# deflect-ca/banjax

Hardware: AMD Instinct MI355X
Metric: log lines/sec matched+rate-limited (node) at 1k rules; HBM GB/s vs peak (higher is better)
Workload: dtype u8

## Files before the change

banjax_amd/csrc/engine.hip:

```cpp
#include <hip/hip_runtime.h>
#include <hipcub/hipcub.hpp>

#include <algorithm>
#include <array>
#include <atomic>
#include <cstdio>
#include <cstdlib>
#include <cstring>
#include <map>
#include <tuple>
#include <memory>
#include <mutex>
#include <stdexcept>
#include <string>
#include <unordered_map>
#include <thread>
#include <vector>

#include "../../include/banjax_gpu.h"
#include "bjx_common.h"
#include "engine_types.h"
#include "regex_compiler.h"
#include "bans.h"

using namespace bjx;

namespace {

struct BjxError : std::runtime_error {
  int code;
  BjxError(int c, const std::string &m) : std::runtime_error(m), code(c) {}
};

#define HIP_OK(expr)                                                                                   \
  do {                                                                                                 \
    hipError_t e_ = (expr);                                                                            \
    if (e_ != hipSuccess)                                                                              \
      throw BjxError(BJX_ERR_DEVICE, std::string(#expr " failed: ") + hipGetErrorString(e_));          \
  } while (0)

constexpr int kBlock = 256;



__device__ __forceinline__ uint32_t nl_mask_word(uint32_t v) {
  uint32_t x = v ^ 0x0A0A0A0Au;
  uint32_t t = ((x & 0x7F7F7F7Fu) + 0x7F7F7F7Fu) | x;
  return ~t & 0x80808080u;
}


__device__ __forceinline__ uint32_t find_space(const uint8_t *p, uint32_t i, uint32_t n) {
  while (i < n && p[i] != ' ') ++i;
  return i;
}

__device__ __forceinline__ bool bytes_eq(const uint8_t *a, const uint8_t *b, uint32_t n) {
  uint32_t k = 0;
  for (; k + 4 <= n; k += 4)
    if (ld4(a + k) != ld4(b + k)) return false;
  for (; k < n; ++k)
    if (a[k] != b[k]) return false;
  return true;
}

__device__ __forceinline__ uint4 ip_key16(const uint8_t *ip, uint32_t len) {
  uint32_t w[4];
#pragma unroll
  for (int k = 0; k < 4; ++k) {
    const uint32_t lo = 4u * k;
    const uint32_t m = len <= lo ? 0u : (len >= lo + 4 ? 0xFFFFFFFFu : (1u << (8 * (len - lo))) - 1u);
    w[k] = m ? ld4(ip + lo) & m : 0u;
  }
  w[3] = (w[3] & 0x00FFFFFFu) | ((len < 255 ? len : 255u) << 24);
  return make_uint4(w[0], w[1], w[2], w[3]);
}
__device__ __forceinline__ uint4 ip_key16_bytes(const uint8_t *ip, uint32_t len) {
  uint32_t w[4] = {0, 0, 0, 0};
  for (uint32_t k = 0; k < len && k < 15; ++k) w[k >> 2] |= (uint32_t)ip[k] << (8 * (k & 3));
  w[3] |= (len < 255 ? len : 255u) << 24;
  return make_uint4(w[0], w[1], w[2], w[3]);
}
constexpr uint32_t kIpWords = 12;

template <uint32_t NW>
__device__ __forceinline__ void ip_words(const uint8_t *p, uint32_t n, uint32_t (&w)[NW]) {
  const uint32_t sh = (uint32_t)(reinterpret_cast<uintptr_t>(p) & 3);
  const uint32_t *a = reinterpret_cast<const uint32_t *>(p - sh);
  const uint32_t nw = n ? (sh + n + 3) >> 2 : 0u;
  uint32_t r[NW + 1];
#pragma unroll
  for (uint32_t k = 0; k <= NW; ++k) r[k] = k < nw ? a[k] : 0u;
#pragma unroll
  for (uint32_t k = 0; k < NW; ++k) {
    const uint32_t lo = 4u * k;
    const uint32_t m = n <= lo ? 0u : (n >= lo + 4 ? 0xFFFFFFFFu : (1u << (8 * (n - lo))) - 1u);
    w[k] = __builtin_amdgcn_alignbyte(r[k + 1], r[k], sh) & m;
  }
}
template <uint32_t NW>
__device__ __forceinline__ uint64_t hash_words(const uint32_t (&w)[NW], uint32_t n) {
// ... 348 lines not shown
    } else if (rule_match(B, r, rest, rest_len)) {
      word |= 1ull << (pos & 63);
      ++nres;
      nev += is_skip(B, r, hid) ? 0u : 1u;
    }
    ++pos;
    if ((pos & 63) == 0) { L.mword(j, wi++) = word; word = 0; }
  }
  if (pos & 63) L.mword(j, wi) = word;
  L.counts[j] = ((uint64_t)nres << 32) | nev;
}

__global__ void k_no_line_pass(unsigned long long *slow_count, unsigned long long n) {
  if (threadIdx.x == 0) *slow_count = n;
}

template <bool SLOW>
__global__ __launch_bounds__(kBlock) void k_parse_match(Bind B, const uint8_t *__restrict__ buf,
                                                        const uint64_t *__restrict__ nl, uint64_t n_lines,
                                                        const uint32_t *__restrict__ list, int64_t now_ns, Lines L,
                                                        uint32_t *slow_list, unsigned long long *slow_count, WideList WL) {
  const uint64_t t = (uint64_t)blockIdx.x * blockDim.x + threadIdx.x;
  if (t >= n_lines) return;
  const uint64_t j = SLOW && list ? list[t] : t;
  const uint64_t s = j ? nl[j - 1] + 1 : 0;
  const uint32_t n = (uint32_t)(nl[j] - s);
  parse_and_match<SLOW>(B, buf + s, s, n, j, now_ns, L, slow_list, slow_count, WL);
}


constexpr uint32_t kWT = 4096;
constexpr uint32_t kHalo = 512;
constexpr uint32_t kLineCap = 128;
constexpr uint32_t kHitSlots = 4;
constexpr int kScanWaves = 16;
constexpr uint32_t kTileLds = kWT + kHalo + 16;
constexpr uint32_t kWaveJobs = 64;
constexpr int kScanGroup = 8;
constexpr uint32_t kCandList = 128;
constexpr uint32_t kBanChunks = 8;
constexpr uint64_t kBanChunkMin = 64ull << 20;
constexpr uint32_t kLongList = 64;
constexpr uint32_t kWaveLds = kTileLds + kLineCap * (2 + 2) + kCandList * 4 + kLineCap * 4 + kLongList * 8 + 16;
constexpr uint32_t kNone = 0xFFFFFFFFu;
constexpr uint32_t kScanLdsMax = 160 * 1024;
constexpr uint32_t kLinesImgMax = 16 * 1024;
constexpr uint32_t kLinesHostLdsMax = 6 * 1024;
constexpr uint32_t kLinesTabLdsMax = 10 * 1024;
constexpr uint32_t kLinesBlocksPerCu = 3;
constexpr uint32_t kSpanBytes = 12 * 1024;

__device__ __forceinline__ uint32_t space_mask16(const uint4 v) {
  const uint32_t wv[4] = {v.x, v.y, v.z, v.w};
  uint32_t m16 = 0;
#pragma unroll
  for (int k = 0; k < 4; ++k) {
    const uint32_t x = wv[k] ^ 0x20202020u;
    const uint32_t hb = ~(((x & 0x7F7F7F7Fu) + 0x7F7F7F7Fu) | x) & 0x80808080u;
    m16 |= (((hb >> 7) & 1u) | ((hb >> 14) & 2u) | ((hb >> 21) & 4u) | ((hb >> 28) & 8u)) << (4 * k);
  }
  return m16;
}

__device__ __forceinline__ bool digits4(uint32_t x) {
  return (x & 0xF0F0F0F0u) == 0x30303030u && (((x & 0x0F0F0F0Fu) + 0x06060606u) & 0xF0F0F0F0u) == 0u;
}
__device__ __forceinline__ uint32_t value4(uint32_t x) {
  x -= 0x30303030u;
  x = x * 10u + (x >> 8);
  return (x & 0xFFu) * 100u + ((x >> 16) & 0xFFu);
}
__device__ __forceinline__ int parse_ts_msec(const uint8_t *p, uint32_t n, double *out) {
  if (n != 14) return 1;
  const uint32_t w0 = ld4(p), w1 = ld4(p + 4), w2 = ld4(p + 8), w3 = ld4(p + 12);
  if (!digits4(w0) || !digits4(w1) || (w2 & 0x00FF0000u) != 0x002E0000u || !digits4((w2 & 0xFF00FFFFu) | 0x00300000u) ||
      !digits4((w3 & 0xFFFFu) | 0x30300000u))
    return 1;
  const uint32_t d8 = w2 & 0xFFu, d9 = (w2 >> 8) & 0xFFu, d11 = w2 >> 24, d12 = w3 & 0xFFu, d13 = (w3 >> 8) & 0xFFu;
  const uint64_t ip = (uint64_t)value4(w0) * 1000000ull + value4(w1) * 100u + (d8 - 48u) * 10u + (d9 - 48u);
  const uint64_t m = ip * 1000ull + (d11 - 48u) * 100u + (d12 - 48u) * 10u + (d13 - 48u);
  *out = (double)m / 1000.0;
  return 0;
}

__device__ __forceinline__ uint32_t find_spaces(const uint8_t *p, uint32_t n, uint32_t &sp0, uint32_t &sp1,
                                                uint32_t &sp2, uint32_t &sp3) {
  const uint32_t skip = (uint32_t)(reinterpret_cast<uintptr_t>(p) & 15);
  const uint4 *base = reinterpret_cast<const uint4 *>(p - skip);
  uint32_t ns = 0, c0 = 0;
  if (n + skip >= 64) {
    const uint4 v0 = base[0], v1 = base[1], v2 = base[2], v3 = base[3];
    uint64_t m = (uint64_t)space_mask16(v0) | ((uint64_t)space_mask16(v1) << 16) | ((uint64_t)space_mask16(v2) << 32) |
                 ((uint64_t)space_mask16(v3) << 48);
    m &= ~((1ull << skip) - 1ull);
#pragma unroll
    for (int k = 0; k < 4; ++k) {
      const uint32_t pos = (uint32_t)__ffsll((unsigned long long)m) - 1 - skip;
      const bool has = m != 0;
      m &= m - 1;
      if (k == 0) sp0 = has ? pos : sp0;
      if (k == 1) sp1 = has ? pos : sp1;
      if (k == 2) sp2 = has ? pos : sp2;
      if (k == 3) sp3 = has ? pos : sp3;
      ns += has ? 1u : 0u;
    }
    c0 = 4;
  }
  for (uint32_t c = c0; c * 16 < n + skip && ns < 4; ++c) {
    const uint4 v = base[c];
    uint32_t m16 = 0;
    const uint32_t wv[4] = {v.x, v.y, v.z, v.w};
#pragma unroll
    for (int k = 0; k < 4; ++k) {
      const uint32_t x = wv[k] ^ 0x20202020u;
      const uint32_t hb = ~(((x & 0x7F7F7F7Fu) + 0x7F7F7F7Fu) | x) & 0x80808080u;
      m16 |= (((hb >> 7) & 1u) | ((hb >> 14) & 2u) | ((hb >> 21) & 4u) | ((hb >> 28) & 8u)) << (4 * k);
    }
    const int32_t lo = (int32_t)skip - (int32_t)(c * 16), hi = lo + (int32_t)n;
    if (lo > 0) m16 &= ~((1u << lo) - 1u);
    if (hi < 16) m16 &= hi > 0 ? (1u << hi) - 1u : 0u;
    while (m16 && ns < 4) {
      const uint32_t pos = c * 16 + (uint32_t)__ffs(m16) - 1 - skip;
      m16 &= m16 - 1;
      sp0 = ns == 0 ? pos : sp0;
      sp1 = ns == 1 ? pos : sp1;
      sp2 = ns == 2 ? pos : sp2;
      sp3 = ns == 3 ? pos : sp3;
      ++ns;
    }
  }
  return ns;
}

struct ScanArgs {
  const uint8_t *buf;
  uint64_t n;
  uint64_t n_tiles;
  uint64_t n_lines;
  const uint64_t *tile_base;
  uint64_t *nl;
  Lines L;
  unsigned long long *stats;
  uint32_t shared_bytes;
  uint32_t debug_skip;
};

__global__ __launch_bounds__(kBlock) void k_nl_count_wt(const uint8_t *__restrict__ buf, uint64_t n, uint64_t n_tiles,
                                                        uint32_t *__restrict__ counts) {
  const uint64_t t = (uint64_t)blockIdx.x * (kBlock / 64) + (threadIdx.x >> 6);
  if (t >= n_tiles) return;
  const uint32_t lane = threadIdx.x & 63;
  const uint64_t base = t * kWT + lane * 64u;
  uint32_t c = 0;
  if (base + 64 <= n) {
    const uint4 *src = reinterpret_cast<const uint4 *>(buf + base);
#pragma unroll
    for (int k = 0; k < 4; ++k) {
      const uint4 v = src[k];
      c += __popc(nl_mask_word(v.x)) + __popc(nl_mask_word(v.y)) + __popc(nl_mask_word(v.z)) + __popc(nl_mask_word(v.w));
    }
  } else {
    for (uint64_t k = base; k < n && k < base + 64; ++k) c += buf[k] == '\n';
  }
  for (int o = 32; o > 0; o >>= 1) c += __shfl_xor(c, o);
  if (lane == 0) counts[t] = c;
}

__device__ __forceinline__ void push_list(uint32_t *list, unsigned long long *count, uint64_t j) {
  const unsigned long long k = atomicAdd(count, 1ull);
  list[k] = (uint32_t)j;
// ... 1561 lines not shown
    const uint32_t aw = acc ? acc[st] : 0u;
    if (aw >> 31) {
      for (;;) {
        uint32_t m = accel_mask(v, aw) & ~((1u << skip) - 1u);
        if (end - a < 16) m &= (1u << (uint32_t)(end - a)) - 1u;
        if (m) { skip = (uint32_t)__ffs(m) - 1; break; }
        a += 16;
        skip = 0;
        if (a >= end) return B.accept_end[R.ae_off + st] != 0;
        v = load16(a);
      }
    }
    const uint4 vn = a + 16 < end ? load16(a + 16) : make_uint4(0, 0, 0, 0);
    const uint32_t wv[4] = {v.x, v.y, v.z, v.w};
    const uint32_t lim = end - a < 16 ? (uint32_t)(end - a) : 16u;
#pragma unroll
    for (uint32_t k = 0; k < 16; ++k) {
      if (k < skip || k >= lim) continue;
      const uint32_t b = (wv[k >> 2] >> (8 * (k & 3))) & 0xFF;
      if (b >= 0x80) {
        const DevRule *Rp = &R;
        uint64_t i = a + k;
        while (i < end) {
          int w;
          const int32_t rune = decode_rune_hd(buf + i, (uint32_t)(end - i), &w);
          uint32_t c;
          if (rune < 0x80) c = ac[rune];
          else {
            const uint32_t *na = B.nonascii + 2 * Rp->na_off;
            uint32_t lo = 0, hi = Rp->n_na;
            while (hi - lo > 1) {
              const uint32_t m = (lo + hi) >> 1;
              if (na[2 * m] <= (uint32_t)rune) lo = m; else hi = m;
            }
            c = na[2 * lo + 1];
          }
          i += (uint32_t)w;
          st = tr[st * ncls + c];
          if (st <= 1) break;
        }
        return B.accept_end[R.ae_off + st] != 0;
      }
      st = tr[st * ncls + ac[b]];
      if (st <= 1) return st == kAccept;
    }
    skip = 0;
    a += 16;
    v = vn;
  }
  return B.accept_end[R.ae_off + st] != 0;
}

__device__ __forceinline__ uint32_t nl_mask16(const uint4 v) {
  const uint32_t wv[4] = {v.x, v.y, v.z, v.w};
  uint32_t m = 0;
#pragma unroll
  for (int q = 0; q < 4; ++q) {
    const uint32_t hb = nl_mask_word(wv[q]);
    m |= (((hb >> 7) & 1u) | ((hb >> 14) & 2u) | ((hb >> 21) & 4u) | ((hb >> 28) & 8u)) << (4 * q);
  }
  return m;
}
template <bool STAGED>
__device__ __forceinline__ bool dfa_line(const Bind &B, const DevRule &R, const uint16_t *tr, const uint8_t *ac,
                                         const uint32_t *acc, const uint8_t *__restrict__ buf, uint64_t n_buf, uint64_t t0,
                                         uint32_t st0) {
  const uint32_t ncls = R.ncls;
  uint32_t st = st0;
  uint64_t a = t0 & ~15ull;
  uint32_t skip = (uint32_t)(t0 - a);
  auto load16 = [&](uint64_t p) -> uint4 {
    if (p + 16 <= n_buf) return *reinterpret_cast<const uint4 *>(buf + p);
    uint32_t w[4];
    for (int k = 0; k < 4; ++k) {
      uint32_t x = 0;
      for (int b = 0; b < 4; ++b) x |= (p + 4 * k + b < n_buf ? (uint32_t)buf[p + 4 * k + b] : 0x0Au) << (8 * b);
      w[k] = x;
    }
    return make_uint4(w[0], w[1], w[2], w[3]);
  };
  uint4 v = load16(a);
  for (;;) {
    uint32_t nlm = nl_mask16(v) & ~((1u << skip) - 1u);
    const uint32_t aw = acc ? acc[st] : 0u;
    if ((aw >> 31) && !nlm) {
      for (;;) {
        const uint32_t m = accel_mask(v, aw) & ~((1u << skip) - 1u);
        if (m || nlm) {
          const uint32_t f = (uint32_t)__ffs(m | nlm) - 1;
          skip = f;
          break;
        }
        a += 16;
        skip = 0;
        v = load16(a);
        nlm = nl_mask16(v);
      }
    } else if (aw >> 31) {
      const uint32_t m = (accel_mask(v, aw) | nlm) & ~((1u << skip) - 1u);
      skip = (uint32_t)__ffs(m) - 1;
    }
    const uint32_t lim = nlm ? (uint32_t)__ffs(nlm) - 1 : 16u;
    const uint4 vn = lim == 16u ? load16(a + 16) : make_uint4(0, 0, 0, 0);
    const uint32_t wv[4] = {v.x, v.y, v.z, v.w};
#pragma unroll
    for (uint32_t k = 0; k < 16; ++k) {
      if (k < skip || k >= lim) continue;
      const uint32_t b = (wv[k >> 2] >> (8 * (k & 3))) & 0xFF;
      if (b >= 0x80) {
        uint64_t i = a + k, end = i;
        while (end < n_buf && buf[end] != '\n') ++end;
        while (i < end) {
          int w;
          const int32_t rune = decode_rune_hd(buf + i, (uint32_t)(end - i), &w);
// ... 4396 lines not shown
                          reinterpret_cast<const void *>(&k_lines<false, false, true>)})
      HIP_OK(hipFuncSetAttribute(f, hipFuncAttributeMaxDynamicSharedMemorySize, (int)kScanLdsMax));
    e->lines_attr = true;
  }
  auto resident_grid = [&](const void *fn, uint32_t lds, uint64_t work) {
    int per_cu = 0;
    HIP_OK(hipOccupancyMaxActiveBlocksPerMultiprocessor(&per_cu, fn, kBlock, lds));
    const uint64_t resident = (uint64_t)std::max(1, per_cu) * (uint64_t)std::max(1, n_cu);
    return (unsigned)std::max<uint64_t>(1, std::min<uint64_t>((work + kBlock - 1) / kBlock, resident));
  };
  for (int attempt = 0;; ++attempt) {
    LinesArgs A;
    A.buf = buf; A.n = n; A.nl = e->nl.p; A.n_lines = n_lines; A.L = L; A.now_ns = now_ns;
    A.dbg = getenv("BJX_DEBUG_LINES") ? (uint32_t)atoi(getenv("BJX_DEBUG_LINES")) : 0u;
    A.dbg2 = getenv("BJX_DEBUG_L2") ? (uint32_t)atoi(getenv("BJX_DEBUG_L2")) : 0u;
    A.slow_list = e->slow_list.p; A.slow_count = e->scalars.p;
    A.jline = e->jline.p; A.jkey = e->jkey.p; A.jidx = e->jidx.p; A.jrec = e->jrec.p; A.job_count = e->scalars.p + 11;
    A.job_cap = std::min(std::min(e->jline.n, e->jkey.n), std::min(e->jidx.n, e->jrec.n));
    A.job_real = e->scalars.p + 14;
    A.null_key = 2 * B.n_rules;
    A.span_bytes = getenv("BJX_SPAN_BYTES") ? (uint32_t)atoi(getenv("BJX_SPAN_BYTES")) & ~15u : kSpanBytes;
    A.list = nullptr; A.n_list = 0; A.prof = nullptr;
    HIP_OK(hipEventRecord(e->evk[0], st));
    static const int lines_env = getenv("BJX_LINES") ? atoi(getenv("BJX_LINES")) : 2;
    const bool use_l2 = B.l2_bytes && lines_env != 1 && !getenv("BJX_PROF_LINES") && !A.dbg;
    e->last_line_kernel = all_wide ? 3u : use_l2 ? 2u : 1u;
    if (all_wide) {
      hipLaunchKernelGGL(k_no_line_pass, dim3(1), dim3(64), 0, st, e->scalars.p, (unsigned long long)n_lines);
      HIP_OK(hipGetLastError());
    } else if (use_l2) {
      const uint32_t lds = B.l2_bytes + (kL2Block / 64) * kL2WaveLds;
      const void *fn = B.l2_w == 2 ? reinterpret_cast<const void *>(&k_lines2<2>) : reinterpret_cast<const void *>(&k_lines2<1>);
      if (lds != e->lines2_lds || B.l2_w != e->lines2_w) {
        HIP_OK(hipFuncSetAttribute(fn, hipFuncAttributeMaxDynamicSharedMemorySize, (int)lds));
        e->lines2_lds = lds;
        e->lines2_w = B.l2_w;
      }
      int per_cu = 0;
      HIP_OK(hipOccupancyMaxActiveBlocksPerMultiprocessor(&per_cu, fn, kL2Block, lds));
      const uint64_t resident = (uint64_t)std::max(1, per_cu) * (uint64_t)std::max(1, n_cu);
      const unsigned grid = (unsigned)std::max<uint64_t>(1, std::min<uint64_t>((n_lines + kL2Block - 1) / kL2Block, resident));
      static const bool dbg_img = getenv("BJX_DEBUG_IMG") != nullptr;
      if (dbg_img) fprintf(stderr, "[bjx] k_lines2: %u B LDS per block (tables %u), %d blocks per CU, grid %u\n", lds, B.l2_bytes, per_cu, grid);
#ifdef BJX_PROF_L2
      e->chk.ensure(16);
      HIP_OK(hipMemsetAsync(e->chk.p, 0, 128, st));
      A.prof = e->chk.p;
#endif
      if (B.l2_w == 2) hipLaunchKernelGGL(k_lines2<2>, dim3(grid), dim3(kL2Block), lds, st, B, A);
      else hipLaunchKernelGGL(k_lines2<1>, dim3(grid), dim3(kL2Block), lds, st, B, A);
      HIP_OK(hipGetLastError());
#ifdef BJX_PROF_L2
      {
        unsigned long long c[8];
        pin_get(e, c, e->chk.p, 64);
        pin_sync(e);
        double tot = 0;
        for (int k = 0; k < 8; ++k) tot += (double)c[k];
        fprintf(stderr, "[bjx] k_lines2 segments (%% of wave clocks): loads %.1f header %.1f host+allow %.1f hits %.1f "
                "anchored %.1f jobs %.1f stores %.1f flush %.1f\n", 100 * c[0] / tot, 100 * c[1] / tot, 100 * c[2] / tot,
                100 * c[3] / tot, 100 * c[4] / tot, 100 * c[5] / tot, 100 * c[6] / tot, 100 * c[7] / tot);
      }
#endif
    } else {
      const bool img_lds = B.img_bytes <= kLinesImgMax;
      const bool host_lds = B.hl_bytes != 0;
      const uint32_t fixed = ((img_lds ? B.img_bytes : 0) + 15u & ~15u) + (host_lds ? B.hl_bytes + 15u & ~15u : 0u) +
                             (kBlock / 64) * kWaveJobBytes;
      if (A.span_bytes && !getenv("BJX_SPAN_BYTES")) {
        const uint32_t share = (kScanLdsMax / kLinesBlocksPerCu) & ~2047u;
        const uint32_t room = share > fixed ? share - fixed : 0u;
        A.span_bytes = std::min<uint32_t>(kSpanBytes, (room / (kBlock / 64) - 32) & ~15u);
      }
      const uint32_t lds = fixed + (kBlock / 64) * (A.span_bytes ? A.span_bytes + 32 : 0);
      const void *fn = img_lds ? (host_lds ? reinterpret_cast<const void *>(&k_lines<true, false, true>)
                                           : reinterpret_cast<const void *>(&k_lines<true>))
                               : (host_lds ? reinterpret_cast<const void *>(&k_lines<false, false, true>)
                                           : reinterpret_cast<const void *>(&k_lines<false>));
      const unsigned grid = resident_grid(fn, lds, A.list ? A.n_list : n_lines);
      const bool prof = getenv("BJX_PROF_LINES") != nullptr;
      A.prof = nullptr;
      if (prof) {
#ifndef BJX_PROF
        throw BjxError(BJX_ERR_ARG, "BJX_PROF_LINES needs a library built with BJX_PROF=1");
#else
        e->chk.ensure(16);
        HIP_OK(hipMemsetAsync(e->chk.p, 0, 128, st));
        A.prof = e->chk.p;
        if (img_lds && host_lds) hipLaunchKernelGGL((k_lines<true, true, true>), dim3(grid), dim3(kBlock), lds, st, B, A);
        else if (img_lds) hipLaunchKernelGGL((k_lines<true, true>), dim3(grid), dim3(kBlock), lds, st, B, A);
        else if (host_lds) hipLaunchKernelGGL((k_lines<false, true, true>), dim3(grid), dim3(kBlock), lds, st, B, A);
        else hipLaunchKernelGGL((k_lines<false, true>), dim3(grid), dim3(kBlock), lds, st, B, A);
        unsigned long long c[10];
        pin_get(e, c, e->chk.p, 80);
        pin_sync(e);
        double tot = 0;
        for (int k = 0; k < 10; ++k) tot += (double)c[k];
        fprintf(stderr, "[bjx] k_lines segments (%% of wave clocks): loads+staging %.1f header %.1f host %.1f host-rules %.1f "
                "hit-decode %.1f site-walk %.1f global-walk %.1f mask-stores %.1f stores %.1f jobs %.1f\n", 100 * c[0] / tot,
                100 * c[1] / tot, 100 * c[2] / tot, 100 * c[3] / tot, 100 * c[7] / tot, 100 * c[8] / tot, 100 * c[9] / tot,
                100 * c[4] / tot, 100 * c[5] / tot, 100 * c[6] / tot);
#endif
      } else if (img_lds && host_lds) hipLaunchKernelGGL((k_lines<true, false, true>), dim3(grid), dim3(kBlock), lds, st, B, A);
      else if (img_lds) hipLaunchKernelGGL(k_lines<true>, dim3(grid), dim3(kBlock), lds, st, B, A);
      else if (host_lds) hipLaunchKernelGGL((k_lines<false, false, true>), dim3(grid), dim3(kBlock), lds, st, B, A);
      else hipLaunchKernelGGL(k_lines<false>, dim3(grid), dim3(kBlock), lds, st, B, A);
      HIP_OK(hipGetLastError());
    }
    HIP_OK(hipEventRecord(e->evk[1], st));
    pin_get(e, &last_nl, e->nl.p + (n_lines - 1), 8);
    pin_get(e, sc4, e->scalars.p + 8, 32);
    pin_get(e, sc4 + 4, e->scalars.p, 8);
    pin_get(e, &n_jobs, e->scalars.p + 14, 8);
    pin_sync(e);
// ... 1219 lines not shown
```

banjax_amd/csrc/lines2.h:

```cpp

#ifdef BJX_PROF_L2
#define L2P(k)                       \
  do {                               \
    __builtin_amdgcn_s_waitcnt(0);   \
    P.mark(k);                       \
  } while (0)
#else
#define L2P(k) \
  do {         \
  } while (0)
#endif

constexpr uint32_t kL2Win = 112;
constexpr int kL2Block = 512;
constexpr uint32_t kL2WaveLds = 64 * kL2Win + kWaveJobBytes;
constexpr uint32_t kL2TabMax = 20 * 1024;
constexpr uint32_t kL2ChkTmpl = 1, kL2ChkFull = 2;
constexpr uint32_t kL2AncWords = 12;
constexpr uint32_t kL2InlineSteps = 64;
constexpr uint32_t kL2NoStart = 0xFFFFFFFFu;
__host__ __device__ constexpr uint32_t l2_dcls_words(uint32_t w) { return (10 * w + 5 + 3) & ~3u; }
__host__ __device__ constexpr uint32_t l2_row_words(uint32_t w) { return (6 * w + 2 + 3) & ~3u; }

template <int W>
struct L2Mask {
  uint64_t w[W];
};
template <int W>
__device__ __forceinline__ L2Mask<W> l2_ld_mask(const uint32_t *hl, uint32_t at) {
  L2Mask<W> m;
#pragma unroll
  for (int k = 0; k < W; ++k) {
    const uint2 v = *reinterpret_cast<const uint2 *>(hl + at + 2 * k);
    m.w[k] = ((uint64_t)v.y << 32) | v.x;
  }
  return m;
}
template <int W>
__device__ __forceinline__ void l2_or(L2Mask<W> &a, const L2Mask<W> &b) {
#pragma unroll
  for (int k = 0; k < W; ++k) a.w[k] |= b.w[k];
}
template <int W>
__device__ __forceinline__ void l2_set(L2Mask<W> &a, uint32_t p) {
#pragma unroll
  for (int k = 0; k < W; ++k)
    if ((p >> 6) == (uint32_t)k) a.w[k] |= 1ull << (p & 63);
}
template <int W>
__device__ __forceinline__ bool l2_has(const L2Mask<W> &a, uint32_t p) {
  bool r = false;
#pragma unroll
  for (int k = 0; k < W; ++k)
    if ((p >> 6) == (uint32_t)k) r = (a.w[k] >> (p & 63)) & 1;
  return r;
}

__device__ __forceinline__ void l2_take_spaces(uint64_t m, int32_t base, uint32_t &ns, uint32_t &sp0, uint32_t &sp1,
                                               uint32_t &sp2, uint32_t &sp3) {
#pragma unroll
  for (int k = 0; k < 4; ++k) {
    const bool has = m != 0 && ns < 4;
    const uint32_t pos = (uint32_t)((int32_t)__ffsll((unsigned long long)m) - 1 + base);
    m &= m - 1;
    sp0 = has && ns == 0 ? pos : sp0;
    sp1 = has && ns == 1 ? pos : sp1;
    sp2 = has && ns == 2 ? pos : sp2;
    sp3 = has && ns == 3 ? pos : sp3;
    ns += has ? 1u : 0u;
  }
}

__device__ __forceinline__ uint32_t l2_spaces(const uint8_t *win, uint32_t sk, const uint8_t *gp, uint32_t n, uint32_t &sp0,
                                              uint32_t &sp1, uint32_t &sp2, uint32_t &sp3) {
  const uint4 *w = reinterpret_cast<const uint4 *>(win);
  uint32_t ns = 0;
  {
    const uint4 v0 = w[0], v1 = w[1], v2 = w[2], v3 = w[3];
    uint64_t m = (uint64_t)space_mask16(v0) | ((uint64_t)space_mask16(v1) << 16) | ((uint64_t)space_mask16(v2) << 32) |
                 ((uint64_t)space_mask16(v3) << 48);
    m &= ~((1ull << sk) - 1ull);
    if (sk + n < 64) m &= (1ull << (sk + n)) - 1ull;
    l2_take_spaces(m, -(int32_t)sk, ns, sp0, sp1, sp2, sp3);
  }
  if (ns < 4 && sk + n > 64) {
    const uint4 v4 = w[4], v5 = w[5], v6 = w[6];
    uint64_t m = (uint64_t)space_mask16(v4) | ((uint64_t)space_mask16(v5) << 16) | ((uint64_t)space_mask16(v6) << 32);
    if (sk + n < kL2Win) m &= (1ull << (sk + n - 64)) - 1ull;
    l2_take_spaces(m, 64 - (int32_t)sk, ns, sp0, sp1, sp2, sp3);
  }
  const uint32_t lim = kL2Win - sk;
  if (ns < 4 && n > lim) {
    uint32_t q0 = 0, q1 = 0, q2 = 0, q3 = 0;
    const uint32_t nq = find_spaces(gp + lim, n - lim, q0, q1, q2, q3);
    const uint32_t q[4] = {q0, q1, q2, q3};
#pragma unroll
    for (uint32_t k = 0; k < 4; ++k) {
      const bool has = k < nq && ns < 4;
      const uint32_t pos = q[k] + lim;
      sp0 = has && ns == 0 ? pos : sp0;
      sp1 = has && ns == 1 ? pos : sp1;
      sp2 = has && ns == 2 ? pos : sp2;
      sp3 = has && ns == 3 ? pos : sp3;
      ns += has ? 1u : 0u;
    }
  }
  return ns;
}

struct L2Line {
  const uint8_t *wp;
  const uint8_t *gp;
  uint32_t lim;
  uint32_t n;
};
__device__ __forceinline__ bool l2_in(const L2Line &X, uint32_t o, uint32_t len) { return o + len + 8 <= X.lim; }

template <bool LDS_TEXT>
__device__ __forceinline__ uint32_t l2_anchored(const Bind &B, const Tabs &T, const LdsTabs &LT, const uint4 a, const uint4 b,
                                                uint32_t r, const uint8_t *rest, uint32_t rest_len, uint32_t host_rel,
                                                uint32_t host_len) {
  const uint32_t kind = (a.x >> 27) & 7u;
  const bool eq = ((a.x >> 30) & 1u) != 0;
  if (kind == kPlanScan) return 2;
  if (kind == kPlanAnchorT) {
    if (!tmpl_at(LT, a.w, rest, rest_len, host_rel, host_len, 0)) return 0;
    return eq ? 1u : 2u;
  }
  const uint4 qa = make_uint4(a.y, a.z, b.x, b.y), qb = make_uint4(b.z, b.w, 0, 0);
  const uint32_t qk = anchor_quick(qa, qb, rest, rest_len);
  if (qk == 0) return 0;
  if (qk == 1 && ((qa.y >> 9) & 1)) return 1;
  if (a.w) {
    if (!((a.w >> 16) <= rest_len && literal_at(T, (a.w & 0xFFFFu) - 1, rest))) return 0;
    return eq ? 1u : 2u;
  }
  const DevRule &R = B.rules[r];
  if (R.anc_len) {
    bool any = false;
    for (uint32_t i = 0; i < R.anc_len && !any; ++i) {
      const uint32_t lit = B.rule_lits[R.anc_off + i];
      any = lit_len_of(T, lit) <= rest_len && literal_at(T, lit, rest);
    }
    if (!any) return 0;
    if (R.anc_equiv) return 1;
  }
  return 2;
}

template <bool LDS_TEXT>
__device__ __forceinline__ uint32_t l2_check(const Tabs &T, const LdsTabs &LT, const uint4 ck, const uint8_t *rest,
                                             uint32_t rest_len, uint32_t host_rel, uint32_t host_len, uint32_t hp) {
  const uint32_t kind = (ck.x >> 8) & 3u;
  const bool eq = ((ck.x >> 10) & 1u) != 0;
  if (kind == kL2ChkTmpl) {
    const uint4 rec = LT.trec[ck.y];
    const uint32_t la = rec.x & 0xFF;
    const bool side_c = ((rec.x >> 16) & 1u) != 0;
// ... 104 lines not shown
    uint4 v = make_uint4(0, 0, 0, 0);
    if (16 - al <= X.n + 1 - o) v = *reinterpret_cast<const uint4 *>(X.gp + o - al);
    else {
      uint32_t t[4] = {0, 0, 0, 0};
      for (uint32_t k = al; k < 16 && o + (k - al) <= X.n; ++k) t[k >> 2] |= (uint32_t)X.gp[o + (k - al)] << (8 * (k & 3));
      v = make_uint4(t[0], t[1], t[2], t[3]);
    }
    const uint32_t w[4] = {v.x, v.y, v.z, v.w};
    for (uint32_t k = al; k < 16 && o < end; ++k, ++o) {
      const uint32_t b = (w[k >> 2] >> (8 * (k & 3))) & 0xFFu;
      if (b >= 0x80) return 2;
      st = tr[st * 128u + b];
      if (st <= 1) return st == kAccept ? 1u : 0u;
    }
  }
  if (o < X.n) return 2;
  return ae[st] ? 1u : 0u;
}

template <int W>
__global__ __launch_bounds__(kL2Block, 4) void k_lines2(Bind B, LinesArgs A) {
  constexpr uint32_t DW = l2_dcls_words(W), RW = l2_row_words(W);
  uint32_t *s_hl = reinterpret_cast<uint32_t *>(s_dyn);
  for (uint32_t i = threadIdx.x; i < B.l2_bytes / 16; i += blockDim.x)
    reinterpret_cast<uint4 *>(s_hl)[i] = reinterpret_cast<const uint4 *>(B.hl)[i];
  __syncthreads();
  const uint32_t lane = threadIdx.x & 63, wave = threadIdx.x >> 6;
  uint8_t *wbase = s_dyn + B.l2_bytes + wave * kL2WaveLds;
  uint8_t *win = wbase + lane * kL2Win;
  JobSink S;
  S.lds = reinterpret_cast<uint4 *>(wbase + 64 * kL2Win);
  S.cnt = reinterpret_cast<uint32_t *>(S.lds + kWaveJobs);
  S.jline = A.jline;
  S.jkey = A.jkey;
  S.jidx = A.jidx;
  S.jrec = A.jrec;
  S.n_rules = B.n_rules;
  S.count = A.job_count;
  S.cap = A.job_cap;
  if (lane == 0) *S.cnt = 0;
  wave_sync();
  JobChunk JC;
  const Tabs TB = make_tabs(B.img, B.il);
  LdsTabs LT;
  LT.hinfo = reinterpret_cast<const uint2 *>(s_hl + B.lt_hinfo);
  LT.cls = reinterpret_cast<const uint4 *>(s_hl + B.lt_cls);
  LT.trec = reinterpret_cast<const uint4 *>(s_hl + B.lt_trec);
  LT.pool = reinterpret_cast<const uint8_t *>(s_hl + B.lt_pool);
  const Lines &L = A.L;
  const uint64_t stride = (uint64_t)gridDim.x * blockDim.x;
#ifdef BJX_PROF_L2
  LinesProf P;
  P.start();
#endif
  for (uint64_t base = (uint64_t)blockIdx.x * blockDim.x + wave * 64u; base < A.n_lines; base += stride) {
    const uint64_t j = base + lane;
    const bool act = j < A.n_lines;
    uint64_t s = 0;
    uint32_t n = 0;
    CandMeta cm{0, 0, 0};
    uint64_t cv[kCandSlots] = {0, 0, 0, 0};
    if (act) {
      s = j ? A.nl[j - 1] + 1 : 0;
      n = (uint32_t)(A.nl[j] - s);
      if (B.any_prefilter) cm = L.cand_meta[j];
    }
    const uint64_t a0 = s & ~15ull;
    const uint32_t sk = (uint32_t)(s - a0);
    {
      uint4 v[kL2Win / 16];
#ifdef BJX_L2_TLOAD
      const uint64_t w0 = __shfl(a0, 0);
      const uint32_t rel = (uint32_t)(a0 - w0);
#pragma unroll
      for (uint32_t k = 0; k < kL2Win / 16; ++k) {
        const uint32_t g = 64u * k + lane;
        const uint32_t ln = (g * 9363u) >> 16;
        const uint64_t a = w0 + __shfl(rel, (int)ln) + 16ull * (g - 7u * ln);
#else
#pragma unroll
      for (uint32_t k = 0; k < kL2Win / 16; ++k) {
        const uint64_t a = a0 + 16ull * k;
#endif
        if (a + 16 <= A.n) v[k] = *reinterpret_cast<const uint4 *>(A.buf + a);
        else {
          uint32_t w4[4];
#pragma unroll
          for (int q = 0; q < 4; ++q) {
            uint32_t x = 0;
            for (int bb = 0; bb < 4; ++bb) {
              const uint64_t p = a + 4 * q + bb;
              if (p < A.n) x |= (uint32_t)A.buf[p] << (8 * bb);
            }
            w4[q] = x;
          }
          v[k] = make_uint4(w4[0], w4[1], w4[2], w4[3]);
        }
      }
      if (act && B.any_prefilter && cm.cnt) {
        const ulonglong2 *cp = reinterpret_cast<const ulonglong2 *>(L.cand + j * kCandSlots);
        const ulonglong2 w0 = cp[0];
        cv[0] = w0.x;
        cv[1] = w0.y;
        if (cm.cnt > 2) {
          const ulonglong2 w1 = cp[1];
          cv[2] = w1.x;
          cv[3] = w1.y;
        }
      }
#ifdef BJX_L2_TLOAD
#pragma unroll
      for (uint32_t k = 0; k < kL2Win / 16; ++k) reinterpret_cast<uint4 *>(wbase)[64u * k + lane] = v[k];
      wave_sync();
#else
#pragma unroll
      for (uint32_t k = 0; k < kL2Win / 16; ++k) reinterpret_cast<uint4 *>(win)[k] = v[k];
#endif
    }
    L2P(0);
    if (act) {
      L2Line X;
      X.wp = win + sk;
      X.gp = A.buf + s;
      X.lim = kL2Win - sk;
      X.n = n;
      uint32_t sp0 = 0, sp1 = 0, sp2 = 0, sp3 = 0;
      const uint32_t ns = l2_spaces(win, sk, X.gp, n, sp0, sp1, sp2, sp3);
      double f = 0.0;
      bool slow = false;
      if (ns >= 4) slow = parse_ts_msec(X.wp, sp0, &f) != 0 && parse_float_fast(X.wp, sp0, &f) != 0;
      L2P(1);
      if (ns < 4) {
        L.flags[j] = kLineError;
        L.counts[j] = 0;
      } else if (slow) {
        L.flags[j] = kLineSlowTs;
        L.counts[j] = 0;
        push_list(A.slow_list, A.slow_count, j);
      } else {
        const uint32_t ip_off = sp0 + 1, ip_len = sp1 - sp0 - 1;
        const uint32_t rest_off = sp1 + 1, host_off = sp2 + 1, host_len = sp3 - sp2 - 1;
        const bool hostw = l2_in(X, host_off, host_len);
        const int32_t hid = hostw ? host_lookup_lds(s_hl, X.wp + host_off, host_len)
                                  : host_lookup_lds(s_hl, X.gp + host_off, host_len);
        const uint32_t dc = hid >= 0 ? s_hl[B.l2_hdc + (uint32_t)hid] : B.l2_none;
        const uint32_t dw = B.l2_dcls + dc * DW;
        const uint32_t rows = s_hl[dw + 10 * W], prule = s_hl[dw + 10 * W + 1], anc = s_hl[dw + 10 * W + 2],
                       n_anc = s_hl[dw + 10 * W + 3];
        const uint32_t first_rule = hid >= 0 ? LT.hinfo[hid].y : 0u;
        const uint32_t pinl = s_hl[dw + 10 * W + 4];
        const bool exempt = B.any_allow && check_is_allowed(B, hid, X.gp + ip_off, ip_len);
        L2P(2);
        const int64_t tsn = ns_from_seconds(f);
        uint8_t fl = 0;
        if (go_sub(A.now_ns, tsn) > 10000000000LL) fl = kLineOld;
        else if (exempt) fl = kLineExempt;
        const uint32_t rest_len = n - rest_off, host_rel = host_off - rest_off;
        L2Mask<W> m = l2_ld_mask<W>(s_hl, dw), J;
#pragma unroll
        for (int k = 0; k < W; ++k) J.w[k] = 0;
        bool evl = false;
        if (fl) {
          L.counts[j] = 0;
        } else {
          const uint32_t cc = cm.cnt;
          const bool ovf = cc > (uint32_t)kCandSlots;
          const uint64_t rs = s + rest_off;
          uint32_t ovbits = 0;
          L2Mask<W> done;
#pragma unroll
          for (int k = 0; k < W; ++k) done.w[k] = 0;
          uint32_t nlit = 0;
#pragma unroll
          for (uint32_t c = 0; c < (uint32_t)kCandSlots; ++c) {
            if (c >= cc || (A.dbg2 & 2)) break;
            const uint64_t v = cv[c];
            const uint32_t lit = (uint32_t)(v & 0x7FFFFF);
            const uint64_t q = v >> 24;
            if (q < rs) continue;
            if (!(v & kCandVerified)) {
              const uint32_t o = (uint32_t)(q - s), ll = lit_len_of(TB, lit);
              if (o + ll > n) continue;
              if (!(l2_in(X, o, ll) ? literal_at(TB, lit, X.wp + o) : literal_at(TB, lit, X.gp + o))) continue;
            }
            if (lit < 32) ovbits |= 1u << lit;
            ++nlit;
            if (ovf) continue;
            const uint32_t hp = q - rs < 0xFFFF ? (uint32_t)(q - rs) : 0xFFFFu;
            const uint32_t rw = rows + lit * RW;
            l2_or(m, l2_ld_mask<W>(s_hl, rw));
            l2_or(J, l2_ld_mask<W>(s_hl, rw + 2 * W));
            const uint32_t ck_off = s_hl[rw + 6 * W], n_ck = s_hl[rw + 6 * W + 1];
            for (uint32_t k = 0; k < n_ck; ++k) {
              const uint4 ck = l2_ld4w(s_hl, ck_off + 4 * k);
              const uint32_t bit = ck.x & 0xFFu;
              if (l2_has(done, bit)) continue;
              uint32_t out;
              if (hp == 0xFFFFu) out = 2;
              else {
                const uint32_t tail = ck.w + (((ck.x >> 11) & 1u) ? host_len : 0u);
                const bool inw = hostw && rest_off + hp + tail + 8 <= X.lim;
                out = inw ? l2_check<true>(TB, LT, ck, X.wp + rest_off, rest_len, host_rel, host_len, hp)
                          : l2_check<false>(TB, LT, ck, X.gp + rest_off, rest_len, host_rel, host_len, hp);
              }
              if (out) {
                l2_set(done, bit);
                if (out == 1) l2_set(m, bit);
                else l2_set(J, bit);
              }
            }
          }
          if (ovf) {
            ovbits |= (uint32_t)(cm.bits & 0xFFFFFFFFull);
            uint32_t ob = ovbits;
            while (ob) {
              const uint32_t l = (uint32_t)__ffs(ob) - 1;
              ob &= ob - 1;
              l2_or(J, l2_ld_mask<W>(s_hl, rows + l * RW + 4 * W));
            }
            l2_or(J, l2_ld_mask<W>(s_hl, dw + 6 * W));
            l2_or(J, l2_ld_mask<W>(s_hl, dw + 8 * W));
          } else if (nlit) {
            l2_or(J, l2_ld_mask<W>(s_hl, dw + 4 * W));
          }
          L2P(3);
          const uint32_t na = (A.dbg2 & 1) ? 0u : n_anc;
          for (uint32_t i = 0; i < na; ++i) {
            const uint32_t ew = anc + kL2AncWords * i;
            const uint4 a = l2_ld4w(s_hl, ew), bq = l2_ld4w(s_hl, ew + 4);
            const uint32_t ext = s_hl[ew + 8];
            const uint32_t pos = (a.x >> 20) & 0x7Fu;
            const uint32_t r = (a.x & kPlanOwn) ? first_rule + pos : (a.x & 0xFFFFFu);
            const uint32_t need = (ext & 0x7FFFFFFFu) + ((ext >> 31) ? host_len : 0u);
            const bool inw = hostw && rest_off + need + 8 <= X.lim;
            const uint32_t out = inw ? l2_anchored<true>(B, TB, LT, a, bq, r, X.wp + rest_off, rest_len, host_rel, host_len)
                                     : l2_anchored<false>(B, TB, LT, a, bq, r, X.gp + rest_off, rest_len, host_rel, host_len);
            if (out == 1) l2_set(m, pos);
            else if (out == 2) l2_set(J, pos);
          }
          L2P(4);
          const L2Mask<W> skp = l2_ld_mask<W>(s_hl, dw + 2 * W);
#pragma unroll
          for (int k = 0; k < W; ++k) {
            J.w[k] &= ~m.w[k];
            evl = evl || ((m.w[k] | J.w[k]) & ~skp.w[k]) != 0;
          }
#pragma unroll
          for (int k = 0; k < W; ++k) {
            uint64_t Jk = (A.dbg2 & 4) ? 0ull : J.w[k];
            while (Jk) {
              const uint32_t p = 64u * k + (uint32_t)__ffsll((unsigned long long)Jk) - 1;
              Jk &= Jk - 1;
              const uint32_t w = s_hl[prule + p];
              const uint32_t r = (w & kPlanOwn) ? first_rule + p : (w & 0xFFFFFu);
              const uint64_t rec = l2_job_rec(B, r, cm, cv, rs, rest_len, rest_off,
                                              B.cfirst ? L.cand_first + j * kCandFirstLits : nullptr);
              uint32_t res = 2;
              if (rec == kJobDecided) res = 1;
              else if (pinl && !(rec & kJobLegacy)) {
                const uint32_t ent = s_hl[pinl + p];
                if (ent) res = l2_inline(s_hl, ent, X, s, rec);
              }
              if (res == 1) m.w[k] |= 1ull << (p & 63);
              else if (res == 2) emit_job(S, j, r, p, rec | (((skp.w[k] >> (p & 63)) & 1) ? kJobNoCount : 0ull));
            }
          }
          L2P(5);
          uint32_t n_m = 0, n_ev = 0;
#pragma unroll
          for (int k = 0; k < W; ++k) {
            L.mword(j, k) = m.w[k];
            n_m += __popcll(m.w[k]);
            n_ev += __popcll(m.w[k] & ~skp.w[k]);
          }
          if (W == 1 && B.mask_words > 1) L.mword(j, 1) = 0;
          L.counts[j] = ((uint64_t)n_m << 32) | (uint64_t)n_ev;
        }
        L.rest_off[j] = rest_off;
        L.host_id[j] = hid;
        L.ip_len[j] = evl ? ip_len : 0u;
        if (evl && !(A.dbg2 & 8)) {
          uint4 k16;
          uint64_t h;
          if (l2_in(X, ip_off, ip_len > 16 ? ip_len : 16u)) ip_key_hash(X.wp + ip_off, ip_len, k16, h);
          else ip_key_hash(X.gp + ip_off, ip_len, k16, h);
          if (ip_len > 15) L.ip_hash[j] = h;
          L.ip16[j] = k16;
        }
        L.ts[j] = tsn;
        L.flags[j] = fl;
      }
    }
    L2P(6);
    flush_jobs(S, JC, lane);
    L2P(7);
  }
  close_jobs(S, JC, lane, A.null_key, A.job_real);
#ifdef BJX_PROF_L2
  if (lane == 0 && A.prof)
    for (int k = 0; k < 8; ++k) atomicAdd(&A.prof[k], (unsigned long long)P.acc[k]);
#endif
}
```

Before: 2.532 billion.

## Simplify lines2 window loads, use udot4 flag masks, route long-header lines to slow path

Replaces the per-byte bit-gathering in space and newline mask computation with udot4-based packing of high-bit flags into a 16-bit mask. The lines2 window load gets a wave-uniform fast path that does seven unconditional 16-byte loads when the whole window is in bounds, with a byte-wise fallback only for the tail. Lines whose first four fields do not fit in the window are now sent to the slow path instead of scanning global memory for spaces, which lets host lookup, allow check and IP hashing always read from the window. Profiling census counters are added under a debug flag. The main risk is behavioural: long headers now take the slow path, and correctness depends on ip and host fields always lying inside the window once four spaces are found there.

Measured after the change: 2.567 billion (median of 6 runs). +1.4%, better.

```diff
diff --git a/banjax_amd/csrc/engine.hip b/banjax_amd/csrc/engine.hip
--- a/banjax_amd/csrc/engine.hip
+++ b/banjax_amd/csrc/engine.hip
@@ -47,6 +47,11 @@
   uint32_t x = v ^ 0x0A0A0A0Au;
   uint32_t t = ((x & 0x7F7F7F7Fu) + 0x7F7F7F7Fu) | x;
   return ~t & 0x80808080u;
+}
+__device__ __forceinline__ uint32_t flag_mask16(uint32_t f0, uint32_t f1, uint32_t f2, uint32_t f3) {
+  const uint32_t a = __builtin_amdgcn_udot4(f1, 0x80402010u, __builtin_amdgcn_udot4(f0, 0x08040201u, 0u, false), false);
+  const uint32_t b = __builtin_amdgcn_udot4(f3, 0x80402010u, __builtin_amdgcn_udot4(f2, 0x08040201u, 0u, false), false);
+  return ((b << 8) | a) >> 7;
 }
 
 
@@ -501,14 +506,13 @@
 
 __device__ __forceinline__ uint32_t space_mask16(const uint4 v) {
   const uint32_t wv[4] = {v.x, v.y, v.z, v.w};
-  uint32_t m16 = 0;
+  uint32_t hb[4];
 #pragma unroll
   for (int k = 0; k < 4; ++k) {
     const uint32_t x = wv[k] ^ 0x20202020u;
-    const uint32_t hb = ~(((x & 0x7F7F7F7Fu) + 0x7F7F7F7Fu) | x) & 0x80808080u;
-    m16 |= (((hb >> 7) & 1u) | ((hb >> 14) & 2u) | ((hb >> 21) & 4u) | ((hb >> 28) & 8u)) << (4 * k);
-  }
-  return m16;
+    hb[k] = ~(((x & 0x7F7F7F7Fu) + 0x7F7F7F7Fu) | x) & 0x80808080u;
+  }
+  return flag_mask16(hb[0], hb[1], hb[2], hb[3]);
 }
 
 __device__ __forceinline__ bool digits4(uint32_t x) {
@@ -557,14 +561,7 @@
   }
   for (uint32_t c = c0; c * 16 < n + skip && ns < 4; ++c) {
     const uint4 v = base[c];
-    uint32_t m16 = 0;
-    const uint32_t wv[4] = {v.x, v.y, v.z, v.w};
-#pragma unroll
-    for (int k = 0; k < 4; ++k) {
-      const uint32_t x = wv[k] ^ 0x20202020u;
-      const uint32_t hb = ~(((x & 0x7F7F7F7Fu) + 0x7F7F7F7Fu) | x) & 0x80808080u;
-      m16 |= (((hb >> 7) & 1u) | ((hb >> 14) & 2u) | ((hb >> 21) & 4u) | ((hb >> 28) & 8u)) << (4 * k);
-    }
+    uint32_t m16 = space_mask16(v);
     const int32_t lo = (int32_t)skip - (int32_t)(c * 16), hi = lo + (int32_t)n;
     if (lo > 0) m16 &= ~((1u << lo) - 1u);
     if (hi < 16) m16 &= hi > 0 ? (1u << hi) - 1u : 0u;
@@ -2232,14 +2229,7 @@
 }
 
 __device__ __forceinline__ uint32_t nl_mask16(const uint4 v) {
-  const uint32_t wv[4] = {v.x, v.y, v.z, v.w};
-  uint32_t m = 0;
-#pragma unroll
-  for (int q = 0; q < 4; ++q) {
-    const uint32_t hb = nl_mask_word(wv[q]);
-    m |= (((hb >> 7) & 1u) | ((hb >> 14) & 2u) | ((hb >> 21) & 4u) | ((hb >> 28) & 8u)) << (4 * q);
-  }
-  return m;
+  return flag_mask16(nl_mask_word(v.x), nl_mask_word(v.y), nl_mask_word(v.z), nl_mask_word(v.w));
 }
 template <bool STAGED>
 __device__ __forceinline__ bool dfa_line(const Bind &B, const DevRule &R, const uint16_t *tr, const uint8_t *ac,
@@ -6742,14 +6732,17 @@
       HIP_OK(hipGetLastError());
 #ifdef BJX_PROF_L2
       {
-        unsigned long long c[8];
-        pin_get(e, c, e->chk.p, 64);
+        unsigned long long c[16];
+        pin_get(e, c, e->chk.p, 128);
         pin_sync(e);
         double tot = 0;
         for (int k = 0; k < 8; ++k) tot += (double)c[k];
         fprintf(stderr, "[bjx] k_lines2 segments (%% of wave clocks): loads %.1f header %.1f host+allow %.1f hits %.1f "
                 "anchored %.1f jobs %.1f stores %.1f flush %.1f\n", 100 * c[0] / tot, 100 * c[1] / tot, 100 * c[2] / tot,
                 100 * c[3] / tot, 100 * c[4] / tot, 100 * c[5] / tot, 100 * c[6] / tot, 100 * c[7] / tot);
+        fprintf(stderr, "[bjx] k_lines2 census of %llu lines, lines / 64-line trips: header past the window %llu / %llu, "
+                "check from HBM %llu / %llu, anchored entry from HBM %llu / %llu, unverified hit from HBM %llu / %llu\n",
+                (unsigned long long)n_lines, c[8], c[9], c[10], c[11], c[12], c[13], c[14], c[15]);
       }
 #endif
     } else {
diff --git a/banjax_amd/csrc/lines2.h b/banjax_amd/csrc/lines2.h
--- a/banjax_amd/csrc/lines2.h
+++ b/banjax_amd/csrc/lines2.h
@@ -71,8 +71,8 @@
   }
 }
 
-__device__ __forceinline__ uint32_t l2_spaces(const uint8_t *win, uint32_t sk, const uint8_t *gp, uint32_t n, uint32_t &sp0,
-                                              uint32_t &sp1, uint32_t &sp2, uint32_t &sp3) {
+__device__ __forceinline__ uint32_t l2_spaces(const uint8_t *win, uint32_t sk, uint32_t n, uint32_t &sp0, uint32_t &sp1,
+                                              uint32_t &sp2, uint32_t &sp3) {
   const uint4 *w = reinterpret_cast<const uint4 *>(win);
   uint32_t ns = 0;
   {
@@ -88,22 +88,6 @@
     uint64_t m = (uint64_t)space_mask16(v4) | ((uint64_t)space_mask16(v5) << 16) | ((uint64_t)space_mask16(v6) << 32);
     if (sk + n < kL2Win) m &= (1ull << (sk + n - 64)) - 1ull;
     l2_take_spaces(m, 64 - (int32_t)sk, ns, sp0, sp1, sp2, sp3);
-  }
-  const uint32_t lim = kL2Win - sk;
-  if (ns < 4 && n > lim) {
-    uint32_t q0 = 0, q1 = 0, q2 = 0, q3 = 0;
-    const uint32_t nq = find_spaces(gp + lim, n - lim, q0, q1, q2, q3);
-    const uint32_t q[4] = {q0, q1, q2, q3};
-#pragma unroll
-    for (uint32_t k = 0; k < 4; ++k) {
-      const bool has = k < nq && ns < 4;
-      const uint32_t pos = q[k] + lim;
-      sp0 = has && ns == 0 ? pos : sp0;
-      sp1 = has && ns == 1 ? pos : sp1;
-      sp2 = has && ns == 2 ? pos : sp2;
-      sp3 = has && ns == 3 ? pos : sp3;
-      ns += has ? 1u : 0u;
-    }
   }
   return ns;
 }
@@ -314,6 +298,7 @@
 #ifdef BJX_PROF_L2
   LinesProf P;
   P.start();
+  unsigned long long cen[8] = {0, 0, 0, 0, 0, 0, 0, 0};
 #endif
   for (uint64_t base = (uint64_t)blockIdx.x * blockDim.x + wave * 64u; base < A.n_lines; base += stride) {
     const uint64_t j = base + lane;
@@ -329,36 +314,8 @@
     }
     const uint64_t a0 = s & ~15ull;
     const uint32_t sk = (uint32_t)(s - a0);
-    {
-      uint4 v[kL2Win / 16];
-#ifdef BJX_L2_TLOAD
-      const uint64_t w0 = __shfl(a0, 0);
-      const uint32_t rel = (uint32_t)(a0 - w0);
-#pragma unroll
-      for (uint32_t k = 0; k < kL2Win / 16; ++k) {
-        const uint32_t g = 64u * k + lane;
-        const uint32_t ln = (g * 9363u) >> 16;
-        const uint64_t a = w0 + __shfl(rel, (int)ln) + 16ull * (g - 7u * ln);
-#else
-#pragma unroll
-      for (uint32_t k = 0; k < kL2Win / 16; ++k) {
-        const uint64_t a = a0 + 16ull * k;
-#endif
-        if (a + 16 <= A.n) v[k] = *reinterpret_cast<const uint4 *>(A.buf + a);
-        else {
-          uint32_t w4[4];
-#pragma unroll
-          for (int q = 0; q < 4; ++q) {
-            uint32_t x = 0;
-            for (int bb = 0; bb < 4; ++bb) {
-              const uint64_t p = a + 4 * q + bb;
-              if (p < A.n) x |= (uint32_t)A.buf[p] << (8 * bb);
-            }
-            w4[q] = x;
-          }
-          v[k] = make_uint4(w4[0], w4[1], w4[2], w4[3]);
-        }
-      }
+    const bool full = __ballot(a0 + kL2Win > A.n) == 0;
+    auto load_cands = [&]() __attribute__((always_inline)) {
       if (act && B.any_prefilter && cm.cnt) {
         const ulonglong2 *cp = reinterpret_cast<const ulonglong2 *>(L.cand + j * kCandSlots);
         const ulonglong2 w0 = cp[0];
@@ -370,16 +327,51 @@
           cv[3] = w1.y;
         }
       }
+    };
+    if (__builtin_expect(full, 1)) {
 #ifdef BJX_L2_TLOAD
+      uint4 v[kL2Win / 16];
+      const uint64_t w0 = __shfl(a0, 0);
+      const uint32_t rel = (uint32_t)(a0 - w0);
+#pragma unroll
+      for (uint32_t k = 0; k < kL2Win / 16; ++k) {
+        const uint32_t g = 64u * k + lane;
+        const uint32_t ln = (g * 9363u) >> 16;
+        const uint64_t a = w0 + __shfl(rel, (int)ln) + 16ull * (g - 7u * ln);
+        v[k] = *reinterpret_cast<const uint4 *>(A.buf + a);
+      }
+      load_cands();
+      __builtin_amdgcn_sched_barrier(0);
 #pragma unroll
       for (uint32_t k = 0; k < kL2Win / 16; ++k) reinterpret_cast<uint4 *>(wbase)[64u * k + lane] = v[k];
-      wave_sync();
 #else
-#pragma unroll
-      for (uint32_t k = 0; k < kL2Win / 16; ++k) reinterpret_cast<uint4 *>(win)[k] = v[k];
-#endif
-    }
+      const uint4 *src = reinterpret_cast<const uint4 *>(A.buf + a0);
+      const uint4 v0 = src[0], v1 = src[1], v2 = src[2], v3 = src[3], v4 = src[4], v5 = src[5], v6 = src[6];
+      load_cands();
+      __builtin_amdgcn_sched_barrier(0);
+      uint4 *dst = reinterpret_cast<uint4 *>(win);
+      dst[0] = v0, dst[1] = v1, dst[2] = v2, dst[3] = v3, dst[4] = v4, dst[5] = v5, dst[6] = v6;
+#endif
+    } else {
+      load_cands();
+#pragma nounroll
+      for (uint32_t q = 0; q < kL2Win / 4; ++q) {
+        uint32_t x = 0;
+#pragma nounroll
+        for (uint32_t bb = 0; bb < 4; ++bb) {
+          const uint64_t p = a0 + 4 * q + bb;
+          if (p < A.n) x |= (uint32_t)A.buf[p] << (8 * bb);
+        }
+        reinterpret_cast<uint32_t *>(win)[q] = x;
+      }
+    }
+#ifdef BJX_L2_TLOAD
+    wave_sync();
+#endif
     L2P(0);
+#ifdef BJX_PROF_L2
+    uint32_t cz = 0;
+#endif
     if (act) {
       L2Line X;
       X.wp = win + sk;
@@ -387,12 +379,15 @@
       X.lim = kL2Win - sk;
       X.n = n;
       uint32_t sp0 = 0, sp1 = 0, sp2 = 0, sp3 = 0;
-      const uint32_t ns = l2_spaces(win, sk, X.gp, n, sp0, sp1, sp2, sp3);
+      const uint32_t ns = l2_spaces(win, sk, n, sp0, sp1, sp2, sp3);
       double f = 0.0;
-      bool slow = false;
+      bool slow = ns < 4 && n > X.lim;
       if (ns >= 4) slow = parse_ts_msec(X.wp, sp0, &f) != 0 && parse_float_fast(X.wp, sp0, &f) != 0;
       L2P(1);
-      if (ns < 4) {
+#ifdef BJX_PROF_L2
+      if (ns < 4 && n > X.lim) cz |= 1u;
+#endif
+      if (ns < 4 && !slow) {
         L.flags[j] = kLineError;
         L.counts[j] = 0;
       } else if (slow) {
@@ -402,16 +397,14 @@
       } else {
         const uint32_t ip_off = sp0 + 1, ip_len = sp1 - sp0 - 1;
         const uint32_t rest_off = sp1 + 1, host_off = sp2 + 1, host_len = sp3 - sp2 - 1;
-        const bool hostw = l2_in(X, host_off, host_len);
-        const int32_t hid = hostw ? host_lookup_lds(s_hl, X.wp + host_off, host_len)
-                                  : host_lookup_lds(s_hl, X.gp + host_off, host_len);
+        const int32_t hid = host_lookup_lds(s_hl, X.wp + host_off, host_len);
         const uint32_t dc = hid >= 0 ? s_hl[B.l2_hdc + (uint32_t)hid] : B.l2_none;
         const uint32_t dw = B.l2_dcls + dc * DW;
         const uint32_t rows = s_hl[dw + 10 * W], prule = s_hl[dw + 10 * W + 1], anc = s_hl[dw + 10 * W + 2],
                        n_anc = s_hl[dw + 10 * W + 3];
         const uint32_t first_rule = hid >= 0 ? LT.hinfo[hid].y : 0u;
         const uint32_t pinl = s_hl[dw + 10 * W + 4];
-        const bool exempt = B.any_allow && check_is_allowed(B, hid, X.gp + ip_off, ip_len);
+        const bool exempt = B.any_allow && check_is_allowed(B, hid, X.wp + ip_off, ip_len);
         L2P(2);
         const int64_t tsn = ns_from_seconds(f);
         uint8_t fl = 0;
@@ -443,6 +436,9 @@
             if (!(v & kCandVerified)) {
               const uint32_t o = (uint32_t)(q - s), ll = lit_len_of(TB, lit);
               if (o + ll > n) continue;
+#ifdef BJX_PROF_L2
+              if (!l2_in(X, o, ll)) cz |= 8u;
+#endif
               if (!(l2_in(X, o, ll) ? literal_at(TB, lit, X.wp + o) : literal_at(TB, lit, X.gp + o))) continue;
             }
             if (lit < 32) ovbits |= 1u << lit;
@@ -461,7 +457,10 @@
               if (hp == 0xFFFFu) out = 2;
               else {
                 const uint32_t tail = ck.w + (((ck.x >> 11) & 1u) ? host_len : 0u);
-                const bool inw = hostw && rest_off + hp + tail + 8 <= X.lim;
+                const bool inw = rest_off + hp + tail + 8 <= X.lim;
+#ifdef BJX_PROF_L2
+                if (!inw) cz |= 2u;
+#endif
                 out = inw ? l2_check<true>(TB, LT, ck, X.wp + rest_off, rest_len, host_rel, host_len, hp)
                           : l2_check<false>(TB, LT, ck, X.gp + rest_off, rest_len, host_rel, host_len, hp);
               }
@@ -494,7 +493,10 @@
             const uint32_t pos = (a.x >> 20) & 0x7Fu;
             const uint32_t r = (a.x & kPlanOwn) ? first_rule + pos : (a.x & 0xFFFFFu);
             const uint32_t need = (ext & 0x7FFFFFFFu) + ((ext >> 31) ? host_len : 0u);
-            const bool inw = hostw && rest_off + need + 8 <= X.lim;
+            const bool inw = rest_off + need + 8 <= X.lim;
+#ifdef BJX_PROF_L2
+            if (!inw) cz |= 4u;
+#endif
             const uint32_t out = inw ? l2_anchored<true>(B, TB, LT, a, bq, r, X.wp + rest_off, rest_len, host_rel, host_len)
                                      : l2_anchored<false>(B, TB, LT, a, bq, r, X.gp + rest_off, rest_len, host_rel, host_len);
             if (out == 1) l2_set(m, pos);
@@ -544,8 +546,7 @@
         if (evl && !(A.dbg2 & 8)) {
           uint4 k16;
           uint64_t h;
-          if (l2_in(X, ip_off, ip_len > 16 ? ip_len : 16u)) ip_key_hash(X.wp + ip_off, ip_len, k16, h);
-          else ip_key_hash(X.gp + ip_off, ip_len, k16, h);
+          ip_key_hash(X.wp + ip_off, ip_len, k16, h);
           if (ip_len > 15) L.ip_hash[j] = h;
           L.ip16[j] = k16;
         }
@@ -556,10 +557,20 @@
     L2P(6);
     flush_jobs(S, JC, lane);
     L2P(7);
+#ifdef BJX_PROF_L2
+    for (int k = 0; k < 4; ++k) {
+      const uint64_t bm = __ballot((cz >> k) & 1u);
+      cen[2 * k] += __popcll(bm);
+      cen[2 * k + 1] += bm != 0;
+    }
+#endif
   }
   close_jobs(S, JC, lane, A.null_key, A.job_real);
 #ifdef BJX_PROF_L2
   if (lane == 0 && A.prof)
-    for (int k = 0; k < 8; ++k) atomicAdd(&A.prof[k], (unsigned long long)P.acc[k]);
-#endif
-}
+    for (int k = 0; k < 8; ++k) {
+      atomicAdd(&A.prof[k], (unsigned long long)P.acc[k]);
+      atomicAdd(&A.prof[8 + k], cen[k]);
+    }
+#endif
+}
```
